# cocowy1/Cost-Volume-Aggregation-in-Stereo-Matching-Revisited

Measured on AMD Instinct MI355X. Metric: cost-volumes/sec (fwd+bwd) at 544x960 D=192, higher is better.
Workload: dtype f32

## Files before the change

### cost-volume-aggregation-in-stereo-matching-revisited_amd/csrc/context_attention.hip

```cpp
#include "dca_common.h"
#include "../../include/dca_hip.h"

__device__ __forceinline__ void class_partials(float val, int kb, bool valid, int n, float* red ,
                                               float* __restrict__ part_row) {
  const int tid = threadIdx.x, wv = tid >> 6, lane = tid & 63;
  for (int k = 0; k < n; ++k) {
    const float s = wave_sum((valid && kb == k) ? val : 0.f);
    if (lane == 0) red[wv * n + k] = s;
  }
  __syncthreads();
  for (int k = tid; k < n; k += 256) part_row[k] = (red[k] + red[n + k]) + (red[2 * n + k] + red[3 * n + k]);
}

__global__ void class_sum_kernel(const float* __restrict__ part, float* __restrict__ out, int nblk, int n, int B) {
  const int i = blockIdx.x * blockDim.x + threadIdx.x;
  if (i >= B * n) return;
  const int b = i / n, k = i % n;
  float s = 0.f;
  for (int j = 0; j < nblk; ++j) s += part[((long)b * nblk + j) * n + k];
  out[i] = s;
}

__global__ __launch_bounds__(256) void ctx_stats_kernel(const float* __restrict__ preds, int* __restrict__ kstar,
                                                        float* __restrict__ e_out, float* __restrict__ pm_out,
// ... 86 lines not shown
                                     const float* __restrict__ denom, const float* __restrict__ dw,
                                     const float* __restrict__ T, float* __restrict__ dpreds, int n, long HW,
                                     long total) {
  for (long idx = (long)blockIdx.x * blockDim.x + threadIdx.x; idx < total; idx += (long)gridDim.x * blockDim.x) {
    const long b = idx / HW, pix = idx % HW;
    const int ks = kstar[idx];
    const float w = e[idx] / denom[b * n + ks];
    const float dm = w * (dw[idx] - T[b * n + ks]);
    const float c0 = dm * pm[idx];
    const float* lp = preds + b * n * HW + pix;
    float* gp = dpreds + b * n * HW + pix;
    float m = -INFINITY;
    for (int k = 0; k < n; ++k) m = fmaxf(m, lp[k * HW]);
    float s = 0.f;
    for (int k = 0; k < n; ++k) s += expf(lp[k * HW] - m);
    const float inv = 1.f / s;
    for (int k = 0; k < n; ++k) {
      const float p = expf(lp[k * HW] - m) * inv;
      gp[k * HW] = c0 * ((k == ks ? 1.f : 0.f) - p);
    }
  }
}

template <int NT, int PW>
__device__ __forceinline__ void attn_stage(const float* const (&src)[NT], float* const (&dst)[NT], long hb, int n, long HW,
                                           long pix0, int tid, int sidx, float scale) {
  constexpr int NTH = 8 * PW, PQ = PW / 4, RQ = 6;
  const int nq = 2 * n * PW;
  if ((HW & 3) == 0 && 8L * n * HW * 4 < 0x7ffffff0L) {
    __amdgpu_buffer_rsrc_t r[NT];
#pragma unroll
    for (int t = 0; t < NT; ++t) r[t] = dca_rsrc(src[t] + hb, 8L * n * HW * 4);
    for (int i0 = 0; i0 < nq; i0 += NTH * RQ) {
      float4 v[NT][RQ];
#pragma unroll
      for (int k = 0; k < RQ; ++k) {
        const int it = i0 + tid + NTH * k, p4 = it & (PQ - 1), cj = it / PQ;
        const int ok = (int)(it < nq) & (int)(pix0 + 4 * p4 < HW);
        const int off = (int)(((long)cj * HW + pix0 + 4 * p4) * 4);
#pragma unroll
        for (int t = 0; t < NT; ++t) v[t][k] = dca_bload4(r[t], off, ok);
      }
#pragma unroll
      for (int k = 0; k < RQ; ++k) {
        const int it = i0 + tid + NTH * k;
        if (it < nq) {
#pragma unroll
          for (int t = 0; t < NT; ++t) {
            float4 w = v[t][k];
            if (t == sidx) { w.x *= scale; w.y *= scale; w.z *= scale; w.w *= scale; }
            *(float4*)(dst[t] + 4 * it) = w;
          }
        }
      }
    }
  } else {
    for (int it = tid; it < 8 * n * PW; it += NTH) {
      const int p = it & (PW - 1), cj = it / PW;
      const bool ok = pix0 + p < HW;
      const long g = hb + (long)cj * HW + pix0 + p;
#pragma unroll
      for (int t = 0; t < NT; ++t) dst[t][it] = ok ? src[t][g] * (t == sidx ? scale : 1.f) : 0.f;
    }
  }
}

template <int QPT, int PW>
__global__ __launch_bounds__(8 * PW) void attn_fwd_kernel(const float* __restrict__ q, const float* __restrict__ k,
                                                       const float* __restrict__ v, float* __restrict__ out, int C,
                                                       int n, long HW) {
  extern __shared__ __attribute__((aligned(16))) float smem[];
  float* ks = smem;
  float* vs = smem + 8 * n * PW;
  const int tid = threadIdx.x, pl = tid & (PW - 1), qg = tid / PW;
  const int head = blockIdx.y, b = blockIdx.z;
  const long pix0 = (long)blockIdx.x * PW, pix = pix0 + pl;
  const long hb = ((long)b * C + head * 8) * n * HW;
  {
    const float* const src[2] = {k, v};
    float* const dst[2] = {ks, vs};
    attn_stage<2, PW>(src, dst, hb, n, HW, pix0, tid, -1, 1.f);
  }
  __syncthreads();
  if (pix >= HW) return;
  float qv[QPT][8], ctx[QPT][8], m[QPT], l[QPT];
#pragma unroll
  for (int t = 0; t < QPT; ++t) {
    const int i = qg + 8 * t;
    m[t] = -INFINITY;
    l[t] = 0.f;
#pragma unroll
    for (int c = 0; c < 8; ++c) {
      qv[t][c] = (i < n) ? q[hb + ((long)c * n + i) * HW + pix] * 0.35355339059327373f : 0.f;
      ctx[t][c] = 0.f;
    }
  }
#pragma unroll 4
  for (int j = 0; j < n; ++j) {
    float kj[8], vj[8];
#pragma unroll
    for (int c = 0; c < 8; ++c) {
      kj[c] = ks[(c * n + j) * PW + pl];
      vj[c] = vs[(c * n + j) * PW + pl];
    }
#pragma unroll
    for (int t = 0; t < QPT; ++t) {
      float s = 0.f;
#pragma unroll
      for (int c = 0; c < 8; ++c) s += qv[t][c] * kj[c];
      const float mn = fmaxf(m[t], s);
      const float corr = expf(m[t] - mn), p = expf(s - mn);
      l[t] = l[t] * corr + p;
#pragma unroll
      for (int c = 0; c < 8; ++c) ctx[t][c] = ctx[t][c] * corr + p * vj[c];
      m[t] = mn;
    }
  }
#pragma unroll
  for (int t = 0; t < QPT; ++t) {
    const int i = qg + 8 * t;
    if (i >= n) continue;
    const float inv = 1.f / l[t];
#pragma unroll
    for (int c = 0; c < 8; ++c) out[hb + ((long)c * n + i) * HW + pix] = ctx[t][c] * inv;
  }
}

template <int QPT, int PW>
__global__ __launch_bounds__(8 * PW) void attn_bwd_kernel(const float* __restrict__ q, const float* __restrict__ k,
                                                       const float* __restrict__ v, const float* __restrict__ dout,
                                                       float* __restrict__ dq, float* __restrict__ dk,
                                                       float* __restrict__ dv, int C, int n, long HW) {
  extern __shared__ __attribute__((aligned(16))) float smem[];
  const int tile = 8 * n * PW;
  float* ks = smem;
  float* vs = smem + tile;
  float* qs = smem + 2 * tile;
  float* gs = smem + 3 * tile;
  float* st = smem + 4 * tile;
  const int tid = threadIdx.x, pl = tid & (PW - 1), qg = tid / PW;
  const int head = blockIdx.y, b = blockIdx.z;
  const long pix0 = (long)blockIdx.x * PW, pix = pix0 + pl;
  const long hb = ((long)b * C + head * 8) * n * HW;
  const float scale = 0.35355339059327373f;
  {
    const float* const src[4] = {k, v, q, dout};
    float* const dst[4] = {ks, vs, qs, gs};
    attn_stage<4, PW>(src, dst, hb, n, HW, pix0, tid, 2, scale);
  }
  __syncthreads();
  {
    float qv[QPT][8], go[QPT][8], dqv[QPT][8], m[QPT], l[QPT], dnum[QPT];
#pragma unroll
    for (int t = 0; t < QPT; ++t) {
      const int i = min(qg + 8 * t, n - 1);
#pragma unroll
      for (int c = 0; c < 8; ++c) {
        qv[t][c] = qs[(c * n + i) * PW + pl];
        go[t][c] = gs[(c * n + i) * PW + pl];
        dqv[t][c] = 0.f;
      }
      m[t] = -INFINITY; l[t] = 0.f; dnum[t] = 0.f;
    }
#pragma unroll 4
    for (int j = 0; j < n; ++j) {
      float kj[8], vj[8];
#pragma unroll
      for (int c = 0; c < 8; ++c) {
        kj[c] = ks[(c * n + j) * PW + pl];
        vj[c] = vs[(c * n + j) * PW + pl];
      }
#pragma unroll
      for (int t = 0; t < QPT; ++t) {
        float s = 0.f, dp = 0.f;
#pragma unroll
        for (int c = 0; c < 8; ++c) {
          s += qv[t][c] * kj[c];
          dp += go[t][c] * vj[c];
        }
        const float mn = fmaxf(m[t], s);
        const float corr = expf(m[t] - mn), p = expf(s - mn);
        l[t] = l[t] * corr + p;
        dnum[t] = dnum[t] * corr + p * dp;
        m[t] = mn;
// ... 21 lines not shown
      }
#pragma unroll
      for (int t = 0; t < QPT; ++t) {
        float s = 0.f, dp = 0.f;
#pragma unroll
        for (int c = 0; c < 8; ++c) {
          s += qv[t][c] * kj[c];
          dp += go[t][c] * vj[c];
        }
        const float ds = expf(s - m[t]) * inv[t] * (dp - Dsum[t]);
#pragma unroll
        for (int c = 0; c < 8; ++c) dqv[t][c] += ds * kj[c];
      }
    }
#pragma unroll
    for (int t = 0; t < QPT; ++t) {
      const int i = qg + 8 * t;
      if (i < n && pix < HW) {
#pragma unroll
        for (int c = 0; c < 8; ++c) dq[hb + ((long)c * n + i) * HW + pix] = dqv[t][c] * scale;
      }
    }
  }
  __syncthreads();
  {
    float kj[QPT][8], vj[QPT][8], dkj[QPT][8], dvj[QPT][8];
#pragma unroll
    for (int t = 0; t < QPT; ++t) {
      const int j = min(qg + 8 * t, n - 1);
#pragma unroll
      for (int c = 0; c < 8; ++c) {
        kj[t][c] = ks[(c * n + j) * PW + pl];
        vj[t][c] = vs[(c * n + j) * PW + pl];
        dkj[t][c] = 0.f;
        dvj[t][c] = 0.f;
      }
    }
#pragma unroll 4
    for (int i = 0; i < n; ++i) {
      float qv[8], go[8];
#pragma unroll
      for (int c = 0; c < 8; ++c) {
        qv[c] = qs[(c * n + i) * PW + pl];
        go[c] = gs[(c * n + i) * PW + pl];
      }
      const float mi = st[(0 * n + i) * PW + pl], li = st[(1 * n + i) * PW + pl], Di = st[(2 * n + i) * PW + pl];
#pragma unroll
      for (int t = 0; t < QPT; ++t) {
        float s = 0.f, dp = 0.f;
#pragma unroll
        for (int c = 0; c < 8; ++c) {
          s += qv[c] * kj[t][c];
          dp += go[c] * vj[t][c];
        }
        const float p = expf(s - mi) * li;
        const float ds = p * (dp - Di);
#pragma unroll
        for (int c = 0; c < 8; ++c) {
          dkj[t][c] += ds * qv[c];
          dvj[t][c] += p * go[c];
        }
      }
    }
#pragma unroll
    for (int t = 0; t < QPT; ++t) {
      const int j = qg + 8 * t;
      if (j < n && pix < HW) {
#pragma unroll
        for (int c = 0; c < 8; ++c) {
          dk[hb + ((long)c * n + j) * HW + pix] = dkj[t][c];
          dv[hb + ((long)c * n + j) * HW + pix] = dvj[t][c];
        }
      }
    }
  }
}

static int ew_grid(long total) {
  long g = (total + 255) / 256;
  return (int)(g < 8192 ? (g > 0 ? g : 1) : 8192);
}

static void ctx_scale_launch(const float* in, const int* kstar, const float* e, const float* denom, float* out, int B, int C,
// ... 16 lines not shown
  hipLaunchKernelGGL(ctx_stats_kernel, dim3(nblk, B), dim3(256), 4 * n * sizeof(float), stream, preds, kstar, e, pm,
                     part, n, HW);
  hipLaunchKernelGGL(class_sum_kernel, dim3(cdiv((long)B * n, 64)), dim3(64), 0, stream, part, denom, nblk, n, B);
  ctx_scale_launch(x, kstar, e, denom, key, B, C, n, HW, stream);
  return dca_launch_status();
}

extern "C" int dca_context_inject_bwd(const float* dkey, const float* x, const float* preds, const int* kstar,
                                      const float* e, const float* pm, const float* denom, float* dx, float* dpreds,
                                      float* dw, float* T, float* part, int B, int C, int n, long HW,
                                      hipStream_t stream) {
  DCA_REQUIRE(dkey && x && preds && kstar && e && pm && denom && dx && dpreds && dw && T && part);
  DCA_REQUIRE(B > 0 && C > 0 && n > 0 && HW > 0 && B <= 65535);
  const int nblk = cdiv(HW, 256);
  hipLaunchKernelGGL(ctx_bwd_reduce_kernel, dim3(nblk, B), dim3(256), 4 * n * sizeof(float), stream, dkey, x, kstar, e,
                     denom, dw, part, C, n, HW);
  hipLaunchKernelGGL(class_sum_kernel, dim3(cdiv((long)B * n, 64)), dim3(64), 0, stream, part, T, nblk, n, B);
  hipLaunchKernelGGL(ctx_bwd_preds_kernel, dim3(ew_grid((long)B * HW)), dim3(256), 0, stream, preds, kstar, e, pm,
                     denom, dw, T, dpreds, n, HW, (long)B * HW);
  ctx_scale_launch(dkey, kstar, e, denom, dx, B, C, n, HW, stream);
  return dca_launch_status();
}

extern "C" int dca_disp_attention_fwd(const float* q, const float* k, const float* v, float* out, int B, int C, int n,
                                      long HW, hipStream_t stream) {
  DCA_REQUIRE(q && k && v && out && B > 0 && C > 0 && C % 8 == 0 && n > 0 && n <= 64 && HW > 0);
  DCA_REQUIRE(C / 8 <= 65535 && B <= 65535);
  const size_t lds = (size_t)2 * 8 * n * 32 * 4;
  const dim3 grid(cdiv(HW, 32), C / 8, B);
  const int qpt = (n + 7) / 8;
#define LAUNCH(Q)                                                                                                      \
  do {                                                                                                                 \
    if (lds > 64 * 1024) {                                                                                             \
      hipError_t e = hipFuncSetAttribute((const void*)attn_fwd_kernel<Q, 32>, hipFuncAttributeMaxDynamicSharedMemorySize, \
                                         (int)lds);                                                                    \
      if (e != hipSuccess) return (int)e;                                                                              \
    }                                                                                                                  \
    hipLaunchKernelGGL((attn_fwd_kernel<Q, 32>), grid, dim3(256), lds, stream, q, k, v, out, C, n, HW);                \
  } while (0)
  switch (qpt) {
    case 1: LAUNCH(1); break;
    case 2: LAUNCH(2); break;
    case 3: LAUNCH(3); break;
    case 4: LAUNCH(4); break;
    case 5: LAUNCH(5); break;
    case 6: LAUNCH(6); break;
    case 7: LAUNCH(7); break;
    default: LAUNCH(8); break;
  }
#undef LAUNCH
  return dca_launch_status();
}

extern "C" int dca_disp_attention_bwd(const float* q, const float* k, const float* v, const float* dout, float* dq,
                                      float* dk, float* dv, int B, int C, int n, long HW, hipStream_t stream) {
  DCA_REQUIRE(q && k && v && dout && dq && dk && dv && B > 0 && C > 0 && C % 8 == 0 && n > 0 && n <= 64 && HW > 0);
  DCA_REQUIRE(C / 8 <= 65535 && B <= 65535);
  const int qpt = (n + 7) / 8;
#define LAUNCH(Q, PWV)                                                                                                 \
  do {                                                                                                                 \
    const size_t lds = (size_t)(4 * 8 + 3) * n * PWV * 4;                                                              \
    const dim3 grid(cdiv(HW, PWV), C / 8, B);                                                                          \
    if (lds > 64 * 1024) {                                                                                             \
      hipError_t e = hipFuncSetAttribute((const void*)attn_bwd_kernel<Q, PWV>,                                         \
                                         hipFuncAttributeMaxDynamicSharedMemorySize, (int)lds);                        \
      if (e != hipSuccess) return (int)e;                                                                              \
    }                                                                                                                  \
    hipLaunchKernelGGL((attn_bwd_kernel<Q, PWV>), grid, dim3(8 * PWV), lds, stream, q, k, v, dout, dq, dk, dv, C, n, HW); \
  } while (0)
  switch (qpt) {
    case 1: LAUNCH(1, 32); break;
    case 2: LAUNCH(2, 32); break;
    case 3: LAUNCH(3, 32); break;
    case 4: LAUNCH(4, 32); break;
    case 5: LAUNCH(5, 16); break;
    case 6: LAUNCH(6, 16); break;
    case 7: LAUNCH(7, 16); break;
    default: LAUNCH(8, 16); break;
  }
#undef LAUNCH
  return dca_launch_status();
}
```

### cost-volume-aggregation-in-stereo-matching-revisited_amd/csrc/dca_common.h

```cpp
#pragma once
#include <hip/hip_runtime.h>
#include <stdint.h>
#include "../../include/dca_hip.h"
#include "dca_tiles.h"

typedef float f32x16 __attribute__((ext_vector_type(16)));
typedef float f32x4 __attribute__((ext_vector_type(4)));

#define DCA_WAVE 64

#define DCA_REQUIRE(cond)                      \
  do {                                         \
    if (!(cond)) return (int)hipErrorInvalidValue; \
  } while (0)

static inline int dca_launch_status() { return (int)hipGetLastError(); }

static inline int cdiv(long a, long b) { return (int)((a + b - 1) / b); }

static inline bool dca_window_ok(int Hc, int Wc, int y0, int rows, int cols) {
  return Hc > 0 && Wc > 0 && (long)Hc * Wc < (1L << 31) && y0 >= 0 && rows > 0 && cols > 0 && (long)y0 + rows <= Hc &&
         cols <= Wc;
}

// ... 13 lines not shown
  int nCxT, nCT, nblk;
  long part_floats;
};
template <int TD, int TH, int TW>
static inline DcaWgradSplitGeom dca_wgrad_split_geometry(int N, int Cx, int Cy, int D, int H, int W) {
  DcaWgradSplitGeom g;
  g.t = dca_tile_grid<TD, TH, TW>(N, D, H, W);
  g.nCxT = cdiv(Cx, 32);
  g.nCT = g.nCxT * cdiv(Cy, 32);
  g.nblk = dca_persistent_grid(g.t.tiles, g.nCT);
  g.part_floats = (long)g.nblk * g.nCT * 27 * 1024;
  return g;
}
int dca_internal_wgrad_reduce(const float* part, float* dw, int nblk, int nCxT, int nCT, int K, int Cy, int Cx, long s_cy,
                              long s_cx, hipStream_t stream);

__device__ __forceinline__ int xcd_remap(int bid, int nwg) {
  const int q = nwg >> 3, r = nwg & 7, xcd = bid & 7, idx = bid >> 3;
  const int base = (xcd < r) ? xcd * (q + 1) : r * (q + 1) + (xcd - r) * q;
  return base + idx;
}

__device__ __forceinline__ float act_apply(float v, float slope) { return v > 0.f ? v : v * slope; }

__device__ __forceinline__ unsigned short dca_sat_u16(float v) {
  if (!(v > 0.f)) return 0;
  if (v >= 65535.f) return 65535;
  return (unsigned short)(unsigned)v;
}

__device__ __forceinline__ float wave_sum(float v) {
#pragma unroll
  for (int o = 32; o > 0; o >>= 1) v += __shfl_xor(v, o, 64);
  return v;
}
__device__ __forceinline__ double wave_sum_d(double v) {
#pragma unroll
  for (int o = 32; o > 0; o >>= 1) v += __shfl_xor(v, o, 64);
  return v;
}
__device__ __forceinline__ float wave_max(float v) {
#pragma unroll
  for (int o = 32; o > 0; o >>= 1) v = fmaxf(v, __shfl_xor(v, o, 64));
  return v;
}

// ... 60 lines not shown
```

### cost-volume-aggregation-in-stereo-matching-revisited_amd/csrc/pointwise.hip

```cpp
#include "dca_frag.h"
#include "../../include/dca_hip.h"

__global__ __launch_bounds__(256) void bn_stats_kernel(const float* __restrict__ x, double* __restrict__ part, int N,
                                                       int C, long S, int nchunk, long chunk_len, int vec) {
  const int c = blockIdx.x, ch = blockIdx.y, tid = threadIdx.x;
  const long s0 = ch * chunk_len, s1 = min(S, s0 + chunk_len);
  const float K = x[(long)c * S];
  if (ch == 0 && tid == 0) part[(long)C * nchunk * 2 + c] = (double)K;
  float s = 0.f, ss = 0.f;
  for (int n = 0; n < N; ++n) {
    const float* p = x + ((long)n * C + c) * S;
    if (vec) {
      for (long i = s0 + 4 * tid; i < s1; i += 1024) {
        float4 v = *(const float4*)(p + i);
        v.x -= K; v.y -= K; v.z -= K; v.w -= K;
        s += (v.x + v.y) + (v.z + v.w);
        ss += (v.x * v.x + v.y * v.y) + (v.z * v.z + v.w * v.w);
      }
    } else {
      for (long i = s0 + tid; i < s1; i += 256) {
        const float v = p[i] - K;
        s += v;
        ss += v * v;
      }
// ... 88 lines not shown
  s = wave_sum_d(s);
  q = wave_sum_d(q);
  const float g = gamma ? gamma[c] : 1.f, b = beta ? beta[c] : 0.f;
  const int ze = zexps ? bn_bound_exp(g, b, n, c, rp_slots, rp_n, rq_slots, rq_n) : 0;
  if (lane != 0) return;
  const double ms = s / n;
  double v = q / n - ms * ms;
  if (v < 0.0) v = 0.0;
  const float mean = (float)(kref + ms), var = (float)v;
  if (running_mean) {
    const double unb = n > 1.0 ? v * n / (n - 1.0) : v;
    running_mean[c] = (1.f - momentum) * running_mean[c] + momentum * mean;
    running_var[c] = (1.f - momentum) * running_var[c] + momentum * (float)unb;
  }
  const float invstd = 1.0f / sqrtf(var + eps);
  stats[c] = mean;
  stats[C + c] = invstd;
  stats[2 * C + c] = g * invstd;
  stats[3 * C + c] = b - mean * g * invstd;
  if (zexps) zexps[c] = ze;
}


__device__ __forceinline__ float bn_affine(float y, float sc, float sh) { return __fmaf_rn(y, sc, sh); }
__device__ __forceinline__ float bn_skip(float y, float sc, float sh) { return act_apply(bn_affine(y, sc, sh), 1.f); }
__device__ __forceinline__ void bn_bwd_acc(float g, float y, float mean, float invstd, float& a0, float& a1) {
#pragma clang fp contract(off)
  a0 += g;
  a1 += g * (y - mean) * invstd;
}

__global__ __launch_bounds__(256) void bn_apply_kernel(const float* __restrict__ y, const float* __restrict__ stats,
                                                       const float* __restrict__ res_pre, const float* __restrict__ res_post,
                                                       float* __restrict__ z, int N, int C, long S, long chunk_len,
                                                       float slope, int vec, unsigned* __restrict__ zmax,
                                                       unsigned* __restrict__ ymax) {
  const int c = blockIdx.y, ch = blockIdx.x, tid = threadIdx.x;
  const long s0 = ch * chunk_len, s1 = min(S, s0 + chunk_len);
  const float mean = stats[c], sc = stats[2 * C + c], sh = stats[3 * C + c];
  float am = 0.f, ym = 0.f;
  for (int n = N - 1; n >= 0; --n) {
    const long base = ((long)n * C + c) * S;
    if (vec) {
      for (long i = s0 + 4 * tid; i < s1; i += 1024) {
        float4 v = *(const float4*)(y + base + i);
        ym = fmaxf(fmaxf(ym, fmaxf(fabsf(v.x - mean), fabsf(v.y - mean))), fmaxf(fabsf(v.z - mean), fabsf(v.w - mean)));
        v.x = bn_affine(v.x, sc, sh); v.y = bn_affine(v.y, sc, sh); v.z = bn_affine(v.z, sc, sh); v.w = bn_affine(v.w, sc, sh);
// ... 1051 lines not shown
```

### cost-volume-aggregation-in-stereo-matching-revisited_amd/models/augment/SelfAttention_bn.py

```python
import torch.nn as nn

from .._bootstrap import ensure as _ensure

ops = _ensure().ops


class _ProjLayer(nn.Sequential):

    def __init__(self, cin, cout):
        super().__init__(nn.Conv3d(cin, cout, kernel_size=1, stride=1, padding=0, bias=False), nn.BatchNorm3d(cout),
                         nn.LeakyReLU(0.1, inplace=True))

    def forward(self, x):
        return ops.convbn3d(x, self[0], self[1], slope=0.1)


class _ProjStack(nn.Sequential):
    def forward(self, x):
        for layer in self:
            x = layer(x)
        return x


class SelfAttentionBlock(nn.Module):

    def __init__(self, key_in_channels, query_in_channels, transform_channels, out_channels, share_key_query,
                 query_downsample, key_downsample, key_query_num_convs, value_out_num_convs, key_query_norm,
                 value_out_norm, matmul_norm, with_out_project, **kwargs):
        super().__init__()
        if (query_downsample is not None or key_downsample is not None or not key_query_norm or not value_out_norm
                or not matmul_norm):
            raise NotImplementedError("only the configuration used by SemanticLevelContext is built")
        self.key_project = self.buildproject(key_in_channels, transform_channels, key_query_num_convs, True)
        if share_key_query:
            assert key_in_channels == query_in_channels
            self.query_project = self.key_project
        else:
            self.query_project = self.buildproject(query_in_channels, transform_channels, key_query_num_convs, True)
        self.value_project = self.buildproject(key_in_channels,
                                               transform_channels if with_out_project else out_channels,
                                               value_out_num_convs, True)
        self.out_project = None
        if with_out_project:
            self.out_project = self.buildproject(transform_channels, out_channels, value_out_num_convs, True)
        self.query_downsample = query_downsample
        self.key_downsample = key_downsample
        self.matmul_norm = matmul_norm
        self.transform_channels = transform_channels

    def forward(self, query_feats, key_feats):
        q = self.query_project(query_feats)
        k = self.key_project(key_feats)
        v = self.value_project(key_feats)
        ctx = ops.disparity_attention(q, k, v)
        if self.out_project is not None:
            ctx = self.out_project(ctx)
        return ctx

    def buildproject(self, in_channels, out_channels, num_convs, use_norm):
        assert use_norm
        convs = [_ProjLayer(in_channels, out_channels)]
        for _ in range(num_convs - 1):
            convs.append(_ProjLayer(out_channels, out_channels))
        if len(convs) > 1:
            return _ProjStack(*convs)
        return convs[0]
```

### cost-volume-aggregation-in-stereo-matching-revisited_amd/ops.py

```python
from __future__ import annotations

import ctypes
import os
import threading

import torch

from ._call import _C, _L, _chk, _ptr, _raw_device, _raw_stream, _req, _req_no_grad, _stream, _vp


def _opt(t, name):
    return None if t is None else _req(t, name)


class _GwcVolume(torch.autograd.Function):
    @staticmethod
    def forward(ctx, ref, tgt, maxdisp, num_groups):
        ref, tgt = _req(ref, "build_gwc_volume"), _req(tgt, "build_gwc_volume")
        B, C, H, W = ref.shape
        vol = torch.empty((B, num_groups, maxdisp, H, W), device=ref.device, dtype=torch.float32)
        with torch.cuda.device_of(ref):
            _chk(_L().dca_gwc_volume_fwd(_ptr(ref), _ptr(tgt), _ptr(vol), B, C, H, W, maxdisp, num_groups, _stream()),
                 "dca_gwc_volume_fwd")
        ctx.save_for_backward(ref, tgt)
# ... 200 lines not shown
        return gl, None


def up_softargmin(logits, scale):
    if logits.shape[1] > 64 or logits.shape[1] < 2 or scale not in (2, 4, 8):
        return softargmin(trilinear_upsample(logits.unsqueeze(1), scale).squeeze(1))
    return _UpSoftArgmin.apply(logits, int(scale))


def _round_up(a, m):
    return (a + m - 1) // m * m


_CONV_MODE = os.environ.get("DCA_CONV", "x2")
CONV_X3 = _CONV_MODE != "fp32"
CONV_X2 = _CONV_MODE == "x2"
WGRAD_S2_X2 = os.environ.get("DCA_WGRAD_S2", "x2") != "fp32"
DECONV_X3 = os.environ.get("DCA_DECONV", "x3") != "fp32"
C1_WGRAD_FUSED = os.environ.get("DCA_C1_WGRAD", "fused") != "expand"
CONV_S2_X2 = os.environ.get("DCA_CONV_S2", "x2") != "fp32"
BN_FUSE = os.environ.get("DCA_BN_FUSE", "1") != "0"
C1_BWD_FUSE = os.environ.get("DCA_C1_BWD", "fused") != "split"
SKIP_FOLD = os.environ.get("DCA_SKIP_FOLD", "1") != "0"
_X3_MIN_WORKGROUPS = 1


AMAX_STATS = {"tagged": 0, "computed": 0, "packed": 0}
CSLOTS = _C["DCA_AMAX_CSLOTS"]
AMAX_EMIT = os.environ.get("DCA_AMAX_EMIT", "1") != "0"
PACK = os.environ.get("DCA_PACK", "1") != "0"


def _cslots(C, device):
    if not AMAX_EMIT:
        return None
    return torch.empty((C * CSLOTS,), device=device, dtype=torch.int32)


def _ver(t):
    return None if t.is_inference() else t._version


def _tag_cmax(t, slots, nslots):
    if slots is not None:
        t._dca_cmax = (slots, int(nslots), _ver(t))
    return t
# ... 165 lines not shown
    gw = torch.empty_like(weight)
    _chk(lib.dca_conv1_bwd_fused(_ptr(dz), _ptr(y), _ptr(stats), _ptr(dgb), float(slope), int(training), _ptr(x), _ptr(x2),
                                 _ptr(weight), _ptr(part), _ptr(gx), _ptr(gx2), _ptr(gw), C1 + C2, 1, N, C1, C2,
                                 weight.shape[0], S, _stream()), "dca_conv1_bwd_fused")
    return gx, gx2, gw


class _SkipBn:
    __slots__ = ("y", "part", "bn", "into")

    def __init__(self, y, part, bn, into):
        self.y, self.part, self.bn, self.into = y, part, bn, into


def _skip_fold_route(x, conv_b, bn_b, slope_b, bn_out):
    if not (SKIP_FOLD and PACK and CONV_X2 and bn_out is not None and torch.is_grad_enabled() and _lp_dtype() is None):
        return "apply"
    C = bn_b.num_features
    if not (bn_b.training and bn_out.training) or bn_out.num_features != C or C % 8 or float(slope_b) != 1.0:
        return "apply"
    if x.dtype != torch.float32 or bn_b.weight is None or bn_b.bias is None:
        return "apply"
    return "fold" if _c1_bwd_route(x, None, conv_b.weight) == "fused" else "apply"


def _k3s1(weight, stride, transposed, x2, head=False):
    return x2 is None and not transposed and int(stride) == 1 and weight.shape[2] == 3 and (weight.shape[0] == 1) == head


def _x2_pairs(xp, yp, W):
    return W % 4 == 0 or (xp and yp)


def _wgrad_family(x, dy, Cx, Cy, ksize, stride):
    Di, Hi, Wi = x.shape[2:]
    Do, Ho, Wo = dy.shape[2:]
    xp, yp = _is_packed(x), _is_packed(dy)
    split = (CONV_X3 and ksize == 3 and x.data_ptr() % 16 == 0 and dy.data_ptr() % 16 == 0
             and max(Cx, Cy) * Di * Hi * Wi * 4 < 0x7ffffff0)
    if split and CONV_X2 and stride == 1 and _x2_pairs(xp, yp, Wi):
        return "x2"
    if xp or yp:
        raise RuntimeError("weight gradient: a packed px2 operand can only feed the f16x2 3x3x3 stride-1 kernel")
    if split and stride == 1 and Wi % 4 == 0:
        return "x3"
    if (split and CONV_X2 and WGRAD_S2_X2 and stride == 2 and Wi % 4 == 0 and Wo % 4 == 0
# ... 811 lines not shown
                             out_dtype=x.dtype)
        xx = _req(x, "convbn3d")
        with torch.cuda.device_of(xx):
            stats = bn_eval_affine(bn)
        C = bn.num_features
        return conv3d_fused_inference(xx, conv.weight, stride, transposed, stats[2 * C:3 * C], stats[3 * C:], slope,
                                      res_pre, res_post, x2)
    if BN_FUSE and bn.training and conv.weight.shape[0 if not transposed else 1] > 1 and _lp_dtype() is None:
        pdy = _pack_dy_ok(x, x2, conv, transposed, stride, res_pre)
        lazy = not transposed and _c1_bwd_route(x, x2, conv.weight, res_pre) == "fused"
        y, part = _Conv3d.apply(x, x2, conv.weight, int(stride), bool(transposed), True, False, pdy, lazy)
        return bn_act(y, bn, slope, res_pre, res_post, part if part.numel() else None, pack_out=pack_out, pack_dy=pdy,
                      lazy_dy=lazy)
    if not transposed and _lp_dtype() is None and _c1_bwd_route(x, x2, conv.weight, res_pre) == "fused":
        y = _Conv3d.apply(x, x2, conv.weight, int(stride), False, False, False, False, True)
        return bn_act(y, bn, slope, res_pre, res_post, lazy_dy=True)
    if _is_packed(x) and _pack_dy_ok(x, x2, conv, transposed, stride, res_pre):
        y = _Conv3d.apply(x, x2, conv.weight, int(stride), bool(transposed), False, False, True)
        return bn_act(y, bn, slope, res_pre, res_post, pack_dy=True)
    y = conv3d(x, conv.weight, stride, transposed, x2)
    return bn_act(y, bn, slope, res_pre, res_post)


class _AvgPool3d(torch.autograd.Function):
    @staticmethod
    def forward(ctx, x):
        x = _req(x, "avg_pool3d")
        N, C, D, H, W = x.shape
        y = torch.empty((N, C, (D + 1) // 2, (H + 1) // 2, (W + 1) // 2), device=x.device, dtype=torch.float32)
        with torch.cuda.device_of(x):
            _chk(_L().dca_avgpool3d_fwd(_ptr(x), _ptr(y), N * C, D, H, W, _stream()), "dca_avgpool3d_fwd")
        ctx.shape = tuple(x.shape)
        return y

    @staticmethod
    def backward(ctx, gy):
        gy = _req(gy, "avg_pool3d.backward")
        N, C, D, H, W = ctx.shape
        gx = torch.empty(ctx.shape, device=gy.device, dtype=torch.float32)
        with torch.cuda.device_of(gy):
            _chk(_L().dca_avgpool3d_bwd(_ptr(gy), _ptr(gx), None, None, N * C, D, H, W, _stream()), "dca_avgpool3d_bwd")
        return gx


class _PoolFork(torch.autograd.Function):

# ... 107 lines not shown
        q, k, v = _req(q, "attention.q"), _req(k, "attention.k"), _req(v, "attention.v")
        B, C, n = q.shape[:3]
        HW = q.shape[3] * q.shape[4]
        out = torch.empty_like(q)
        with torch.cuda.device_of(q):
            _chk(_L().dca_disp_attention_fwd(_ptr(q), _ptr(k), _ptr(v), _ptr(out), B, C, n, HW, _stream()),
                 "dca_disp_attention_fwd")
        ctx.save_for_backward(q, k, v)
        return out

    @staticmethod
    def backward(ctx, dout):
        q, k, v = ctx.saved_tensors
        dout = _req(dout, "attention.backward")
        B, C, n = q.shape[:3]
        HW = q.shape[3] * q.shape[4]
        dq, dk, dv = torch.empty_like(q), torch.empty_like(k), torch.empty_like(v)
        with torch.cuda.device_of(q):
            _chk(_L().dca_disp_attention_bwd(_ptr(q), _ptr(k), _ptr(v), _ptr(dout), _ptr(dq), _ptr(dk), _ptr(dv), B,
                                             C, n, HW, _stream()), "dca_disp_attention_bwd")
        return dq, dk, dv


def context_inject(x, preds):
    return _ContextInject.apply(x, preds)


def disparity_attention(q, k, v):
    if q.dim() != 5 or q.shape[1] % 8 or q.shape[2] > 64:
        raise RuntimeError(f"disparity_attention: needs (B, C % 8 == 0, n <= 64, H, W) tensors, got {tuple(q.shape)} "
                           "(n = maxdisp/8 with the down-sampling cva, maxdisp/4 without)")
    return _DispAttention.apply(q, k, v)


class _ConvexUp4(torch.autograd.Function):
    @staticmethod
    def forward(ctx, mask_logits, disp):
        mask_logits, disp = _req(mask_logits, "convex_upsample4.mask"), _req(disp, "convex_upsample4.disp")
        B, C, h, w = mask_logits.shape
        if C != 144 or tuple(disp.shape) != (B, 1, h, w):
            raise RuntimeError(f"convex_upsample4: expected mask (B,144,h,w) and disp (B,1,h,w), got "
                               f"{tuple(mask_logits.shape)} and {tuple(disp.shape)}")
        up = torch.empty((B, 1, 4 * h, 4 * w), device=disp.device, dtype=torch.float32)
        with torch.cuda.device_of(disp):
            _chk(_L().dca_convex_up4_fwd(_ptr(mask_logits), _ptr(disp), _ptr(up), B, h, w, _stream()),
                 "dca_convex_up4_fwd")
        ctx.save_for_backward(mask_logits, disp)
        return up

    @staticmethod
    def backward(ctx, gup):
        mask_logits, disp = ctx.saved_tensors
        gup = _req(gup, "convex_upsample4.backward")
        B, _, h, w = mask_logits.shape
        gl, gd = torch.empty_like(mask_logits), torch.empty_like(disp)
# ... 271 lines not shown
```

### include/dca_hip.h

```cpp
#ifndef DCA_HIP_H
#define DCA_HIP_H

#include <hip/hip_runtime_api.h>

#ifdef __cplusplus
extern "C" {
#endif

#define DCA_ABI_VERSION 20
int dca_abi_version(void);

#define DCA_BF16 1
#define DCA_FP16 2

int dca_gwc_volume_fwd(const float* ref, const float* tgt, float* vol, int B, int C, int H, int W, int maxdisp,
                       int num_groups, hipStream_t stream);
int dca_gwc_volume_bwd(const float* gvol, const float* ref, const float* tgt, float* gref, float* gtgt, int B, int C,
                       int H, int W, int maxdisp, int num_groups, hipStream_t stream);
int dca_concat_volume_fwd(const float* ref, const float* tgt, float* vol, int B, int C, int H, int W, int maxdisp,
                          hipStream_t stream);
int dca_concat_volume_bwd(const float* gvol, float* gref, float* gtgt, int B, int C, int H, int W, int maxdisp,
                          hipStream_t stream);

int dca_cost_volume_fwd(const float* const* refs, const float* const* tgts, const int* seg_channels, int nseg,
// ... 121 lines not shown
                           unsigned* ymax, const float* y_r, const float* stats_r, const float* res_post, float* zf,
                           unsigned* zmax, hipStream_t stream);
int dca_bn_backward_skip(const float* dz, const float* y, const float* y_r, const float* stats, const float* stats_r,
                         double* part, double* part_r, float* dgb, float* dgb_r, float* dy, float* g_out, int N, int C,
                         long S, float slope, int training, unsigned* dmax, hipStream_t stream);

int dca_avgpool3d_fwd(const float* x, float* y, long NC, int Di, int Hi, int Wi, hipStream_t stream);
int dca_avgpool3d_bwd(const float* gy, float* gx, const float* res, const float* res2, long NC, int Di, int Hi, int Wi,
                     hipStream_t stream);

int dca_trilinear_fwd(const float* x, float* y, long NC, int Di, int Hi, int Wi, int scale, hipStream_t stream);
int dca_trilinear_bwd(const float* gy, float* gx, long NC, int Di, int Hi, int Wi, int scale, hipStream_t stream);

int dca_context_inject_fwd(const float* x, const float* preds, float* key, int* kstar, float* e, float* pm,
                           float* denom, float* part, int B, int C, int n, long HW, hipStream_t stream);
int dca_context_inject_bwd(const float* dkey, const float* x, const float* preds, const int* kstar, const float* e,
                           const float* pm, const float* denom, float* dx, float* dpreds, float* dw, float* T,
                           float* part, int B, int C, int n, long HW, hipStream_t stream);

int dca_disp_attention_fwd(const float* q, const float* k, const float* v, float* out, int B, int C, int n, long HW,
                           hipStream_t stream);
int dca_disp_attention_bwd(const float* q, const float* k, const float* v, const float* dout, float* dq, float* dk,
                           float* dv, int B, int C, int n, long HW, hipStream_t stream);

int dca_convex_up4_fwd(const float* mask_logits, const float* disp, float* up, int B, int h, int w, hipStream_t stream);
int dca_convex_up4_bwd(const float* mask_logits, const float* disp, const float* gup, float* glogits, float* gdisp,
                       float* wk, int B, int h, int w, hipStream_t stream);

long dca_focal_loss_workspace(int nlev, int B, long HW);
int dca_focal_loss_fwd(const float* const* ests, const float* weights, int nlev, const float* gt, double* work,
                       float* out, int B, int K, long HW, float focal_coefficient, hipStream_t stream);
int dca_focal_loss_bwd(const float* const* ests, float* const* gests, const float* weights, int nlev, const float* gt,
                       const double* work, const float* gloss, int B, int K, long HW, float focal_coefficient,
                       hipStream_t stream);

long dca_conv3d_lp_weight_bytes(int Cin, int Cout);
int dca_conv3d_lp_prep_weight(const float* w, void* wx, int A, int B, int src_ab, int flip, int dtype,
                              hipStream_t stream);
int dca_conv3d_lp_forward(const void* x, const void* wx, void* y, const float* scale, const float* shift,
                          const void* res_pre, const void* res_post, float slope, int N, int Cin, int Cout, int D, int H,
                          int W, int dtype, int in_f32, int out_f32, hipStream_t stream);

long dca_conv1_lp_weight_bytes(int C1, int C2);
int dca_conv1_lp_prep_weight(const float* w, void* wfrag, int Cout, int C1, int C2, int dtype, hipStream_t stream);
int dca_conv1_lp_forward(const void* x, const void* x2, const void* wfrag, void* y, const float* scale,
                         const float* shift, const void* res_pre, const void* res_post, float slope, int N, int C1,
// ... 160 lines not shown
```

Measured before the change: 43.69.

## Fold BN+activation of q/k/v projections into disparity attention kernels

The q/k/v projection BatchNorm+LeakyReLU is no longer materialized. The attention forward and backward kernels now apply the BN affine and activation while staging raw conv outputs, and the backward emits pre-activation gradients that feed a BN backward reduce. The backward kernel also reuses LDS by staging q/dout first, then k/v into the same buffers, which cuts shared memory from 4 tiles to 2 and may raise occupancy. This removes three elementwise BN-apply passes and their tensors, at the cost of extra per-element math and more syncs inside the attention kernels.

```diff
diff --git a/cost-volume-aggregation-in-stereo-matching-revisited_amd/csrc/context_attention.hip b/cost-volume-aggregation-in-stereo-matching-revisited_amd/csrc/context_attention.hip
--- a/cost-volume-aggregation-in-stereo-matching-revisited_amd/csrc/context_attention.hip
+++ b/cost-volume-aggregation-in-stereo-matching-revisited_amd/csrc/context_attention.hip
@@ -132,9 +132,34 @@
   }
 }
 
-template <int NT, int PW>
+struct AttnBn {
+  const float* sq;
+  const float* sk;
+  const float* sv;
+  float slope;
+};
+__device__ __forceinline__ float attn_uniform(float x) {
+  return __uint_as_float(__builtin_amdgcn_readfirstlane(__float_as_uint(x)));
+}
+__device__ __forceinline__ float attn_pick(const float* __restrict__ p, int cj, int n) {
+  const float a0 = attn_uniform(p[0]), a1 = attn_uniform(p[1]), a2 = attn_uniform(p[2]), a3 = attn_uniform(p[3]);
+  const float a4 = attn_uniform(p[4]), a5 = attn_uniform(p[5]), a6 = attn_uniform(p[6]), a7 = attn_uniform(p[7]);
+  float r = a0;
+  r = cj >= n ? a1 : r;
+  r = cj >= 2 * n ? a2 : r;
+  r = cj >= 3 * n ? a3 : r;
+  r = cj >= 4 * n ? a4 : r;
+  r = cj >= 5 * n ? a5 : r;
+  r = cj >= 6 * n ? a6 : r;
+  r = cj >= 7 * n ? a7 : r;
+  return r;
+}
+
+template <int NT, int PW, int NB = 0>
 __device__ __forceinline__ void attn_stage(const float* const (&src)[NT], float* const (&dst)[NT], long hb, int n, long HW,
-                                           long pix0, int tid, int sidx, float scale) {
+                                           long pix0, int tid, int sidx, float scale,
+                                           const float* const (&stats)[NB ? NB : 1] = {nullptr}, int C = 0, int head = 0,
+                                           float slope = 1.f) {
   constexpr int NTH = 8 * PW, PQ = PW / 4, RQ = 6;
   const int nq = 2 * n * PW;
   if ((HW & 3) == 0 && 8L * n * HW * 4 < 0x7ffffff0L) {
@@ -155,9 +180,19 @@
       for (int k = 0; k < RQ; ++k) {
         const int it = i0 + tid + NTH * k;
         if (it < nq) {
+          const int cj = it / PQ;
+          const bool in = pix0 + 4 * (it & (PQ - 1)) < HW;
 #pragma unroll
           for (int t = 0; t < NT; ++t) {
             float4 w = v[t][k];
+            if (t < NB) {
+              const float* hs = stats[t] + 2 * C + head * 8;
+              const float sc = attn_pick(hs, cj, n), sh = attn_pick(hs + C, cj, n);
+              w.x = in ? act_apply(bn_affine(w.x, sc, sh), slope) : 0.f;
+              w.y = in ? act_apply(bn_affine(w.y, sc, sh), slope) : 0.f;
+              w.z = in ? act_apply(bn_affine(w.z, sc, sh), slope) : 0.f;
+              w.w = in ? act_apply(bn_affine(w.w, sc, sh), slope) : 0.f;
+            }
             if (t == sidx) { w.x *= scale; w.y *= scale; w.z *= scale; w.w *= scale; }
             *(float4*)(dst[t] + 4 * it) = w;
           }
@@ -170,15 +205,26 @@
       const bool ok = pix0 + p < HW;
       const long g = hb + (long)cj * HW + pix0 + p;
 #pragma unroll
-      for (int t = 0; t < NT; ++t) dst[t][it] = ok ? src[t][g] * (t == sidx ? scale : 1.f) : 0.f;
-    }
-  }
-}
-
-template <int QPT, int PW>
+      for (int t = 0; t < NT; ++t) {
+        float w = 0.f;
+        if (ok) {
+          w = src[t][g];
+          if (t < NB) {
+            const float* hs = stats[t] + 2 * C + head * 8;
+            w = act_apply(bn_affine(w, attn_pick(hs, cj, n), attn_pick(hs + C, cj, n)), slope);
+          }
+          w *= (t == sidx ? scale : 1.f);
+        }
+        dst[t][it] = w;
+      }
+    }
+  }
+}
+
+template <int QPT, int PW, bool BN>
 __global__ __launch_bounds__(8 * PW) void attn_fwd_kernel(const float* __restrict__ q, const float* __restrict__ k,
                                                        const float* __restrict__ v, float* __restrict__ out, int C,
-                                                       int n, long HW) {
+                                                       int n, long HW, AttnBn bn) {
   extern __shared__ __attribute__((aligned(16))) float smem[];
   float* ks = smem;
   float* vs = smem + 8 * n * PW;
@@ -189,7 +235,12 @@
   {
     const float* const src[2] = {k, v};
     float* const dst[2] = {ks, vs};
-    attn_stage<2, PW>(src, dst, hb, n, HW, pix0, tid, -1, 1.f);
+    if constexpr (BN) {
+      const float* const stats[2] = {bn.sk, bn.sv};
+      attn_stage<2, PW, 2>(src, dst, hb, n, HW, pix0, tid, -1, 1.f, stats, C, head, bn.slope);
+    } else {
+      attn_stage<2, PW>(src, dst, hb, n, HW, pix0, tid, -1, 1.f);
+    }
   }
   __syncthreads();
   if (pix >= HW) return;
@@ -201,7 +252,13 @@
     l[t] = 0.f;
 #pragma unroll
     for (int c = 0; c < 8; ++c) {
-      qv[t][c] = (i < n) ? q[hb + ((long)c * n + i) * HW + pix] * 0.35355339059327373f : 0.f;
+      if constexpr (BN) {
+        const float sc = bn.sq[2 * C + head * 8 + c], sh = bn.sq[3 * C + head * 8 + c];
+        qv[t][c] = (i < n) ? act_apply(bn_affine(q[hb + ((long)c * n + i) * HW + pix], sc, sh), bn.slope) * 0.35355339059327373f
+                           : 0.f;
+      } else {
+        qv[t][c] = (i < n) ? q[hb + ((long)c * n + i) * HW + pix] * 0.35355339059327373f : 0.f;
+      }
       ctx[t][c] = 0.f;
     }
   }
@@ -236,40 +293,62 @@
   }
 }
 
-template <int QPT, int PW>
+template <int QPT, int PW, bool BN>
 __global__ __launch_bounds__(8 * PW) void attn_bwd_kernel(const float* __restrict__ q, const float* __restrict__ k,
                                                        const float* __restrict__ v, const float* __restrict__ dout,
                                                        float* __restrict__ dq, float* __restrict__ dk,
-                                                       float* __restrict__ dv, int C, int n, long HW) {
+                                                       float* __restrict__ dv, int C, int n, long HW, AttnBn bn) {
   extern __shared__ __attribute__((aligned(16))) float smem[];
   const int tile = 8 * n * PW;
   float* ks = smem;
   float* vs = smem + tile;
-  float* qs = smem + 2 * tile;
-  float* gs = smem + 3 * tile;
-  float* st = smem + 4 * tile;
+  float* qs = smem;
+  float* gs = smem + tile;
+  float* st = smem + 2 * tile;
   const int tid = threadIdx.x, pl = tid & (PW - 1), qg = tid / PW;
   const int head = blockIdx.y, b = blockIdx.z;
   const long pix0 = (long)blockIdx.x * PW, pix = pix0 + pl;
   const long hb = ((long)b * C + head * 8) * n * HW;
   const float scale = 0.35355339059327373f;
   {
-    const float* const src[4] = {k, v, q, dout};
-    float* const dst[4] = {ks, vs, qs, gs};
-    attn_stage<4, PW>(src, dst, hb, n, HW, pix0, tid, 2, scale);
+    const float* const src[2] = {q, dout};
+    float* const dst[2] = {qs, gs};
+    if constexpr (BN) {
+      const float* const stats[1] = {bn.sq};
+      attn_stage<2, PW, 1>(src, dst, hb, n, HW, pix0, tid, 0, scale, stats, C, head, bn.slope);
+    } else {
+      attn_stage<2, PW>(src, dst, hb, n, HW, pix0, tid, 0, scale);
+    }
+  }
+  __syncthreads();
+  float qv[QPT][8], go[QPT][8];
+#pragma unroll
+  for (int t = 0; t < QPT; ++t) {
+    const int i = min(qg + 8 * t, n - 1);
+#pragma unroll
+    for (int c = 0; c < 8; ++c) {
+      qv[t][c] = qs[(c * n + i) * PW + pl];
+      go[t][c] = gs[(c * n + i) * PW + pl];
+    }
   }
   __syncthreads();
   {
-    float qv[QPT][8], go[QPT][8], dqv[QPT][8], m[QPT], l[QPT], dnum[QPT];
-#pragma unroll
-    for (int t = 0; t < QPT; ++t) {
-      const int i = min(qg + 8 * t, n - 1);
-#pragma unroll
-      for (int c = 0; c < 8; ++c) {
-        qv[t][c] = qs[(c * n + i) * PW + pl];
-        go[t][c] = gs[(c * n + i) * PW + pl];
-        dqv[t][c] = 0.f;
-      }
+    const float* const src[2] = {k, v};
+    float* const dst[2] = {ks, vs};
+    if constexpr (BN) {
+      const float* const stats[2] = {bn.sk, bn.sv};
+      attn_stage<2, PW, 2>(src, dst, hb, n, HW, pix0, tid, -1, 1.f, stats, C, head, bn.slope);
+    } else {
+      attn_stage<2, PW>(src, dst, hb, n, HW, pix0, tid, -1, 1.f);
+    }
+  }
+  __syncthreads();
+  {
+    float dqv[QPT][8], m[QPT], l[QPT], dnum[QPT];
+#pragma unroll
+    for (int t = 0; t < QPT; ++t) {
+#pragma unroll
+      for (int c = 0; c < 8; ++c) dqv[t][c] = 0.f;
       m[t] = -INFINITY; l[t] = 0.f; dnum[t] = 0.f;
     }
 #pragma unroll 4
@@ -337,7 +416,6 @@
       }
     }
   }
-  __syncthreads();
   {
     float kj[QPT][8], vj[QPT][8], dkj[QPT][8], dvj[QPT][8];
 #pragma unroll
@@ -346,18 +424,43 @@
 #pragma unroll
       for (int c = 0; c < 8; ++c) {
         kj[t][c] = ks[(c * n + j) * PW + pl];
+      }
+    }
+    __syncthreads();
+#pragma unroll
+    for (int t = 0; t < QPT; ++t) {
+      const int i = qg + 8 * t, j = min(i, n - 1);
+#pragma unroll
+      for (int c = 0; c < 8; ++c) {
         vj[t][c] = vs[(c * n + j) * PW + pl];
+        if (i < n) qs[(c * n + i) * PW + pl] = qv[t][c];
+      }
+    }
+    __syncthreads();
+#pragma unroll
+    for (int t = 0; t < QPT; ++t) {
+      const int i = qg + 8 * t;
+      if (i < n) {
+#pragma unroll
+        for (int c = 0; c < 8; ++c) gs[(c * n + i) * PW + pl] = go[t][c];
+      }
+    }
+    __syncthreads();
+#pragma unroll
+    for (int t = 0; t < QPT; ++t) {
+#pragma unroll
+      for (int c = 0; c < 8; ++c) {
         dkj[t][c] = 0.f;
         dvj[t][c] = 0.f;
       }
     }
 #pragma unroll 4
     for (int i = 0; i < n; ++i) {
-      float qv[8], go[8];
+      float qi[8], gi[8];
 #pragma unroll
       for (int c = 0; c < 8; ++c) {
-        qv[c] = qs[(c * n + i) * PW + pl];
-        go[c] = gs[(c * n + i) * PW + pl];
+        qi[c] = qs[(c * n + i) * PW + pl];
+        gi[c] = gs[(c * n + i) * PW + pl];
       }
       const float mi = st[(0 * n + i) * PW + pl], li = st[(1 * n + i) * PW + pl], Di = st[(2 * n + i) * PW + pl];
 #pragma unroll
@@ -365,15 +468,15 @@
         float s = 0.f, dp = 0.f;
 #pragma unroll
         for (int c = 0; c < 8; ++c) {
-          s += qv[c] * kj[t][c];
-          dp += go[c] * vj[t][c];
+          s += qi[c] * kj[t][c];
+          dp += gi[c] * vj[t][c];
         }
         const float p = expf(s - mi) * li;
         const float ds = p * (dp - Di);
 #pragma unroll
         for (int c = 0; c < 8; ++c) {
-          dkj[t][c] += ds * qv[c];
-          dvj[t][c] += p * go[c];
+          dkj[t][c] += ds * qi[c];
+          dvj[t][c] += p * gi[c];
         }
       }
     }
@@ -436,21 +539,20 @@
   return dca_launch_status();
 }
 
-extern "C" int dca_disp_attention_fwd(const float* q, const float* k, const float* v, float* out, int B, int C, int n,
-                                      long HW, hipStream_t stream) {
-  DCA_REQUIRE(q && k && v && out && B > 0 && C > 0 && C % 8 == 0 && n > 0 && n <= 64 && HW > 0);
-  DCA_REQUIRE(C / 8 <= 65535 && B <= 65535);
+template <bool BN>
+static int attn_fwd_launch(const float* q, const float* k, const float* v, float* out, AttnBn bn, int B, int C, int n, long HW,
+                           hipStream_t stream) {
   const size_t lds = (size_t)2 * 8 * n * 32 * 4;
   const dim3 grid(cdiv(HW, 32), C / 8, B);
   const int qpt = (n + 7) / 8;
 #define LAUNCH(Q)                                                                                                      \
   do {                                                                                                                 \
     if (lds > 64 * 1024) {                                                                                             \
-      hipError_t e = hipFuncSetAttribute((const void*)attn_fwd_kernel<Q, 32>, hipFuncAttributeMaxDynamicSharedMemorySize, \
-                                         (int)lds);                                                                    \
+      hipError_t e = hipFuncSetAttribute((const void*)attn_fwd_kernel<Q, 32, BN>,                                      \
+                                         hipFuncAttributeMaxDynamicSharedMemorySize, (int)lds);                        \
       if (e != hipSuccess) return (int)e;                                                                              \
     }                                                                                                                  \
-    hipLaunchKernelGGL((attn_fwd_kernel<Q, 32>), grid, dim3(256), lds, stream, q, k, v, out, C, n, HW);                \
+    hipLaunchKernelGGL((attn_fwd_kernel<Q, 32, BN>), grid, dim3(256), lds, stream, q, k, v, out, C, n, HW, bn);        \
   } while (0)
   switch (qpt) {
     case 1: LAUNCH(1); break;
@@ -466,21 +568,21 @@
   return dca_launch_status();
 }
 
-extern "C" int dca_disp_attention_bwd(const float* q, const float* k, const float* v, const float* dout, float* dq,
-                                      float* dk, float* dv, int B, int C, int n, long HW, hipStream_t stream) {
-  DCA_REQUIRE(q && k && v && dout && dq && dk && dv && B > 0 && C > 0 && C % 8 == 0 && n > 0 && n <= 64 && HW > 0);
-  DCA_REQUIRE(C / 8 <= 65535 && B <= 65535);
+template <bool BN>
+static int attn_bwd_launch(const float* q, const float* k, const float* v, const float* dout, float* dq, float* dk, float* dv,
+                           AttnBn bn, int B, int C, int n, long HW, hipStream_t stream) {
   const int qpt = (n + 7) / 8;
 #define LAUNCH(Q, PWV)                                                                                                 \
   do {                                                                                                                 \
-    const size_t lds = (size_t)(4 * 8 + 3) * n * PWV * 4;                                                              \
+    const size_t lds = (size_t)(2 * 8 + 3) * n * PWV * 4;                                                              \
     const dim3 grid(cdiv(HW, PWV), C / 8, B);                                                                          \
     if (lds > 64 * 1024) {                                                                                             \
-      hipError_t e = hipFuncSetAttribute((const void*)attn_bwd_kernel<Q, PWV>,                                         \
+      hipError_t e = hipFuncSetAttribute((const void*)attn_bwd_kernel<Q, PWV, BN>,                                     \
                                          hipFuncAttributeMaxDynamicSharedMemorySize, (int)lds);                        \
       if (e != hipSuccess) return (int)e;                                                                              \
     }                                                                                                                  \
-    hipLaunchKernelGGL((attn_bwd_kernel<Q, PWV>), grid, dim3(8 * PWV), lds, stream, q, k, v, dout, dq, dk, dv, C, n, HW); \
+    hipLaunchKernelGGL((attn_bwd_kernel<Q, PWV, BN>), grid, dim3(8 * PWV), lds, stream, q, k, v, dout, dq, dk, dv, C, n, HW, \
+                       bn);                                                                                            \
   } while (0)
   switch (qpt) {
     case 1: LAUNCH(1, 32); break;
@@ -495,3 +597,36 @@
 #undef LAUNCH
   return dca_launch_status();
 }
+
+#define ATTN_REQUIRE_SHAPE DCA_REQUIRE(B > 0 && C > 0 && C % 8 == 0 && n > 0 && n <= 64 && HW > 0 && C / 8 <= 65535 && B <= 65535)
+
+extern "C" int dca_disp_attention_fwd(const float* q, const float* k, const float* v, float* out, int B, int C, int n,
+                                      long HW, hipStream_t stream) {
+  DCA_REQUIRE(q && k && v && out);
+  ATTN_REQUIRE_SHAPE;
+  return attn_fwd_launch<false>(q, k, v, out, AttnBn{nullptr, nullptr, nullptr, 1.f}, B, C, n, HW, stream);
+}
+
+extern "C" int dca_disp_attention_bwd(const float* q, const float* k, const float* v, const float* dout, float* dq,
+                                      float* dk, float* dv, int B, int C, int n, long HW, hipStream_t stream) {
+  DCA_REQUIRE(q && k && v && dout && dq && dk && dv);
+  ATTN_REQUIRE_SHAPE;
+  return attn_bwd_launch<false>(q, k, v, dout, dq, dk, dv, AttnBn{nullptr, nullptr, nullptr, 1.f}, B, C, n, HW, stream);
+}
+
+extern "C" int dca_disp_attention_bn_fwd(const float* yq, const float* yk, const float* yv, const float* stats_q,
+                                         const float* stats_k, const float* stats_v, float slope, float* out, int B, int C,
+                                         int n, long HW, hipStream_t stream) {
+  DCA_REQUIRE(yq && yk && yv && stats_q && stats_k && stats_v && out);
+  ATTN_REQUIRE_SHAPE;
+  return attn_fwd_launch<true>(yq, yk, yv, out, AttnBn{stats_q, stats_k, stats_v, slope}, B, C, n, HW, stream);
+}
+
+extern "C" int dca_disp_attention_bn_bwd(const float* yq, const float* yk, const float* yv, const float* stats_q,
+                                         const float* stats_k, const float* stats_v, float slope, const float* dout,
+                                         float* dq, float* dk, float* dv, int B, int C, int n, long HW, hipStream_t stream) {
+  DCA_REQUIRE(yq && yk && yv && stats_q && stats_k && stats_v && dout && dq && dk && dv);
+  ATTN_REQUIRE_SHAPE;
+  return attn_bwd_launch<true>(yq, yk, yv, dout, dq, dk, dv, AttnBn{stats_q, stats_k, stats_v, slope}, B, C, n, HW, stream);
+}
+#undef ATTN_REQUIRE_SHAPE
diff --git a/cost-volume-aggregation-in-stereo-matching-revisited_amd/csrc/dca_common.h b/cost-volume-aggregation-in-stereo-matching-revisited_amd/csrc/dca_common.h
--- a/cost-volume-aggregation-in-stereo-matching-revisited_amd/csrc/dca_common.h
+++ b/cost-volume-aggregation-in-stereo-matching-revisited_amd/csrc/dca_common.h
@@ -59,6 +59,8 @@
 }
 
 __device__ __forceinline__ float act_apply(float v, float slope) { return v > 0.f ? v : v * slope; }
+
+__device__ __forceinline__ float bn_affine(float y, float sc, float sh) { return __fmaf_rn(y, sc, sh); }
 
 __device__ __forceinline__ unsigned short dca_sat_u16(float v) {
   if (!(v > 0.f)) return 0;
diff --git a/cost-volume-aggregation-in-stereo-matching-revisited_amd/csrc/pointwise.hip b/cost-volume-aggregation-in-stereo-matching-revisited_amd/csrc/pointwise.hip
--- a/cost-volume-aggregation-in-stereo-matching-revisited_amd/csrc/pointwise.hip
+++ b/cost-volume-aggregation-in-stereo-matching-revisited_amd/csrc/pointwise.hip
@@ -134,7 +134,6 @@
 }
 
 
-__device__ __forceinline__ float bn_affine(float y, float sc, float sh) { return __fmaf_rn(y, sc, sh); }
 __device__ __forceinline__ float bn_skip(float y, float sc, float sh) { return act_apply(bn_affine(y, sc, sh), 1.f); }
 __device__ __forceinline__ void bn_bwd_acc(float g, float y, float mean, float invstd, float& a0, float& a1) {
 #pragma clang fp contract(off)
diff --git a/cost-volume-aggregation-in-stereo-matching-revisited_amd/models/augment/SelfAttention_bn.py b/cost-volume-aggregation-in-stereo-matching-revisited_amd/models/augment/SelfAttention_bn.py
--- a/cost-volume-aggregation-in-stereo-matching-revisited_amd/models/augment/SelfAttention_bn.py
+++ b/cost-volume-aggregation-in-stereo-matching-revisited_amd/models/augment/SelfAttention_bn.py
@@ -14,12 +14,21 @@
     def forward(self, x):
         return ops.convbn3d(x, self[0], self[1], slope=0.1)
 
+    def deferred(self, x):
+        return ops.convbn3d_proj(x, self[0], self[1], slope=0.1)
+
 
 class _ProjStack(nn.Sequential):
     def forward(self, x):
         for layer in self:
             x = layer(x)
         return x
+
+    def deferred(self, x):
+        layers = list(self)
+        for layer in layers[:-1]:
+            x = layer(x)
+        return layers[-1].deferred(x)
 
 
 class SelfAttentionBlock(nn.Module):
@@ -49,10 +58,10 @@
         self.transform_channels = transform_channels
 
     def forward(self, query_feats, key_feats):
-        q = self.query_project(query_feats)
-        k = self.key_project(key_feats)
-        v = self.value_project(key_feats)
-        ctx = ops.disparity_attention(q, k, v)
+        q = self.query_project.deferred(query_feats)
+        k = self.key_project.deferred(key_feats)
+        v = self.value_project.deferred(key_feats)
+        ctx = ops.disparity_attention_proj(q, k, v)
         if self.out_project is not None:
             ctx = self.out_project(ctx)
         return ctx
diff --git a/cost-volume-aggregation-in-stereo-matching-revisited_amd/ops.py b/cost-volume-aggregation-in-stereo-matching-revisited_amd/ops.py
--- a/cost-volume-aggregation-in-stereo-matching-revisited_amd/ops.py
+++ b/cost-volume-aggregation-in-stereo-matching-revisited_amd/ops.py
@@ -246,6 +246,7 @@
 BN_FUSE = os.environ.get("DCA_BN_FUSE", "1") != "0"
 C1_BWD_FUSE = os.environ.get("DCA_C1_BWD", "fused") != "split"
 SKIP_FOLD = os.environ.get("DCA_SKIP_FOLD", "1") != "0"
+ATTN_BN_FOLD = os.environ.get("DCA_ATTN_BN", "1") != "0"
 _X3_MIN_WORKGROUPS = 1
 
 
@@ -457,6 +458,23 @@
     if x.dtype != torch.float32 or bn_b.weight is None or bn_b.bias is None:
         return "apply"
     return "fold" if _c1_bwd_route(x, None, conv_b.weight) == "fused" else "apply"
+
+
+class _ProjBn:
+    __slots__ = ("y", "part", "bn", "slope")
+
+    def __init__(self, y, part, bn, slope):
+        self.y, self.part, self.bn, self.slope = y, part, bn, slope
+
+
+def _attn_bn_route(x, conv, bn):
+    if not (ATTN_BN_FOLD and torch.is_grad_enabled() and _lp_dtype() is None):
+        return "apply"
+    if x.dim() != 5 or x.dtype != torch.float32 or bn.weight is None or bn.bias is None:
+        return "apply"
+    if isinstance(conv, torch.nn.ConvTranspose3d) or conv.stride[0] != 1 or bn.num_features % 8 or x.shape[2] > 64:
+        return "apply"
+    return "fold" if _c1_bwd_route(x, None, conv.weight) == "fused" else "apply"
 
 
 def _k3s1(weight, stride, transposed, x2, head=False):
@@ -1314,6 +1332,16 @@
     return bn_act(y, bn, slope, res_pre, res_post)
 
 
+def convbn3d_proj(x, conv, bn, slope):
+    if _attn_bn_route(x, conv, bn) != "fold":
+        return convbn3d(x, conv, bn, slope)
+    if BN_FUSE and bn.training and conv.weight.shape[0] > 1:
+        y, part = _Conv3d.apply(x, None, conv.weight, 1, False, True, False, False, True)
+        return _ProjBn(y, part if part.numel() else None, bn, float(slope))
+    y = _Conv3d.apply(x, None, conv.weight, 1, False, False, False, False, True)
+    return _ProjBn(y, None, bn, float(slope))
+
+
 class _AvgPool3d(torch.autograd.Function):
     @staticmethod
     def forward(ctx, x):
@@ -1467,6 +1495,51 @@
         return dq, dk, dv
 
 
+class _DispAttentionBn(torch.autograd.Function):
+
+    @staticmethod
+    def forward(ctx, yq, yk, yv, slope, *bns):
+        ys = [_req(y, "attention." + t) for y, t in zip((yq, yk, yv), "qkv")]
+        if not (ys[0].shape == ys[1].shape == ys[2].shape):
+            raise RuntimeError("disparity_attention: q, k and v differ in shape")
+        B, C, n = ys[0].shape[:3]
+        HW = ys[0].shape[3] * ys[0].shape[4]
+        out = torch.empty_like(ys[0])
+        with torch.cuda.device_of(ys[0]):
+            stats = [bn_stats_vector(y, *bns[8 * i:8 * i + 8]) for i, y in enumerate(ys)]
+            _chk(_L().dca_disp_attention_bn_fwd(_ptr(ys[0]), _ptr(ys[1]), _ptr(ys[2]), _ptr(stats[0]), _ptr(stats[1]),
+                                                _ptr(stats[2]), float(slope), _ptr(out), B, C, n, HW, _stream()),
+                 "dca_disp_attention_bn_fwd")
+        ctx.save_for_backward(*ys, *stats)
+        ctx.meta = (float(slope), tuple(bool(bns[8 * i + 4]) for i in range(3)))
+        return out
+
+    @staticmethod
+    def backward(ctx, dout):
+        ys, stats = ctx.saved_tensors[:3], ctx.saved_tensors[3:]
+        slope, training = ctx.meta
+        dout = _req(dout, "attention.backward")
+        N, C, n = ys[0].shape[:3]
+        HW = ys[0].shape[3] * ys[0].shape[4]
+        S = n * HW
+        lib = _L()
+        dzs = [torch.empty_like(y) for y in ys]
+        grads = []
+        with torch.cuda.device_of(ys[0]):
+            _chk(lib.dca_disp_attention_bn_bwd(_ptr(ys[0]), _ptr(ys[1]), _ptr(ys[2]), _ptr(stats[0]), _ptr(stats[1]),
+                                               _ptr(stats[2]), slope, _ptr(dout), _ptr(dzs[0]), _ptr(dzs[1]), _ptr(dzs[2]), N,
+                                               C, n, HW, _stream()), "dca_disp_attention_bn_bwd")
+            nchunk = lib.dca_bn_num_chunks(C, S)
+            for dz, y, st, tr in zip(dzs, ys, stats, training):
+                part = torch.empty((C * nchunk * 2,), device=y.device, dtype=torch.float64)
+                dgb = torch.empty((4 * C,), device=y.device, dtype=torch.float32)
+                _chk(lib.dca_bn_backward_reduce(_ptr(dz), _ptr(y), _ptr(st), _ptr(part), _ptr(dgb), N, C, S, slope, int(tr),
+                                                _stream()), "dca_bn_backward_reduce")
+                dz._dca_lazy = (y, st, dgb, slope, tr)
+                grads += [dgb[:C], dgb[C:2 * C], None, None, None, None, None, None]
+        return (dzs[0], dzs[1], dzs[2], None, *grads)
+
+
 def context_inject(x, preds):
     return _ContextInject.apply(x, preds)
 
@@ -1476,6 +1549,29 @@
         raise RuntimeError(f"disparity_attention: needs (B, C % 8 == 0, n <= 64, H, W) tensors, got {tuple(q.shape)} "
                            "(n = maxdisp/8 with the down-sampling cva, maxdisp/4 without)")
     return _DispAttention.apply(q, k, v)
+
+
+def _proj_applied(p):
+    return bn_act(p.y, p.bn, p.slope, stats_part=p.part, lazy_dy=True) if isinstance(p, _ProjBn) else p
+
+
+def disparity_attention_proj(q, k, v):
+    ps = (q, k, v)
+    fold = all(isinstance(p, _ProjBn) for p in ps)
+    if fold:
+        fold = q.y.shape == k.y.shape == v.y.shape and q.slope == k.slope == v.slope
+    if not fold:
+        return disparity_attention(*[_proj_applied(p) for p in ps])
+    args = []
+    for p in ps:
+        bn = p.bn
+        training = bn.training or bn.running_mean is None
+        args += [bn.weight, bn.bias, bn.running_mean, bn.running_var, training, 0.1 if bn.momentum is None else bn.momentum,
+                 bn.eps, p.part if training else None]
+    out = _DispAttentionBn.apply(q.y, k.y, v.y, q.slope, *args)
+    for p in ps:
+        _bn_count(p.bn)
+    return out
 
 
 class _ConvexUp4(torch.autograd.Function):
diff --git a/include/dca_hip.h b/include/dca_hip.h
--- a/include/dca_hip.h
+++ b/include/dca_hip.h
@@ -167,6 +167,12 @@
                            hipStream_t stream);
 int dca_disp_attention_bwd(const float* q, const float* k, const float* v, const float* dout, float* dq, float* dk,
                            float* dv, int B, int C, int n, long HW, hipStream_t stream);
+int dca_disp_attention_bn_fwd(const float* yq, const float* yk, const float* yv, const float* stats_q, const float* stats_k,
+                              const float* stats_v, float slope, float* out, int B, int C, int n, long HW,
+                              hipStream_t stream);
+int dca_disp_attention_bn_bwd(const float* yq, const float* yk, const float* yv, const float* stats_q, const float* stats_k,
+                              const float* stats_v, float slope, const float* dout, float* dq, float* dk, float* dv, int B,
+                              int C, int n, long HW, hipStream_t stream);
 
 int dca_convex_up4_fwd(const float* mask_logits, const float* disp, float* up, int B, int h, int w, hipStream_t stream);
 int dca_convex_up4_bwd(const float* mask_logits, const float* disp, const float* gup, float* glogits, float* gdisp,
```

Result: no change. 44.04, median of 6 (+0.8%).
